# titus-leistner/mmlf

Hardware: AMD Instinct MI355X
Metric: 96x96 EPI patches/sec fwd+bwd, bs=512 (higher is better)
Workload: dtype f32 via 2 x f16 operand split (22 significant bits per operand, locally scaled; 3 MFMA passes, f32 accumulate)

## Files before the change

### include/mmlf_hip.h

```cpp
#ifndef MMLF_HIP_H
#define MMLF_HIP_H

#include <stddef.h>
#include <stdint.h>

#ifdef __cplusplus
extern "C" {
#endif

#define MMLF_TILE_POSITIONS 256

const char *mmlf_last_error(void);
#define MMLF_ABI_VERSION 10
int mmlf_abi_version(void);

const char *mmlf_build_info(void);
int mmlf_build_is_ablation(void);
int mmlf_conv_cus(void);

enum { MMLF_AUDIT_IN = 0, MMLF_AUDIT_PACKED = 1, MMLF_AUDIT_BIAS = 2, MMLF_AUDIT_OUT = 3, MMLF_AUDIT_REF = 4,
       MMLF_AUDIT_IN_AMAX = 5, MMLF_AUDIT_OUT_AMAX = 6, MMLF_AUDIT_BN_PARTIAL = 7, MMLF_AUDIT_MASK = 8, MMLF_AUDIT_CONV_N = 9 };
int mmlf_audit_conv_h2(int cs_in, int K, int N, int cs_out, int N_store, int out_shift, int cs_ref, int B, int H, int W,
                       int64_t *ends);
enum { MMLF_AUDIT_WG_IN = 0, MMLF_AUDIT_WG_G = 1, MMLF_AUDIT_WG_GW = 2, MMLF_AUDIT_WG_GB = 3, MMLF_AUDIT_WG_WORKSPACE = 4,
       MMLF_AUDIT_WG_IN_AMAX = 5, MMLF_AUDIT_WG_G_AMAX = 6, MMLF_AUDIT_WGRAD_N = 7 };
int mmlf_audit_wgrad_h2(int cs_in, int Cin, int cs_g, int Cout, int g_shift, int B, int H, int W, int64_t *ends);

int64_t mmlf_grid_alloc_positions(int B, int H, int W);
int64_t mmlf_packed_filter_floats(int K, int N);
int64_t mmlf_wgrad_workspace_floats(int Cin, int Cout, int B, int H, int W);

enum { MMLF_VAR_IDENTITY = 0, MMLF_VAR_TRANSPOSE = 1, MMLF_VAR_TRANSPOSE_FLIPH = 2 };

int mmlf_pack_filter(const float *w_oihw, float *packed, int Cout, int Cin, int variant, int dgrad,
                     void *stream);

int mmlf_conv2x2(const float *in, int cs_in, int K, const float *packed, const float *bias, int N,
                 float *out, int cs_out, int N_store, int out_shift, int vh, int vw,
                 int B, int H, int W, int relu, const float *relu_ref, int cs_ref, void *stream);

int64_t mmlf_packed_filter_split_bytes(int K, int N);
int mmlf_pack_filter_split(const float *w_oihw, void *packed, int Cout, int Cin, int variant, int dgrad,
                           void *stream);
int mmlf_conv2x2_split(const float *in, int cs_in, int K, const void *packed, const float *bias, int N,
                       float *out, int cs_out, int N_store, int out_shift, int vh, int vw,
                       int B, int H, int W, int relu, const float *relu_ref, int cs_ref, void *stream);
// ... 155 lines not shown
```

### mmlf_amd/_lib.py

```python
import ctypes
import os
import re

import torch

_HERE = os.path.dirname(os.path.abspath(__file__))
LIB_PATH = os.environ.get('MMLF_HIP_LIB') or os.path.join(_HERE, 'csrc', 'libmmlf_hip.so')

_HEADER = os.path.join(os.path.dirname(_HERE), 'include', 'mmlf_hip.h')
_CTYPES = {'int': ctypes.c_int, 'int32_t': ctypes.c_int32, 'int64_t': ctypes.c_int64, 'long long': ctypes.c_longlong,
           'double': ctypes.c_double, 'float': ctypes.c_float}


def signatures_from_header(text):
    text = re.sub(r'/\*.*?\*/', ' ', text, flags=re.S)
    text = re.sub(r'//[^\n]*', ' ', text)
    text = re.sub(r'^[ \t]*#(?:[^\n]*\\\n)*[^\n]*', ' ', text, flags=re.M)
    text = re.sub(r'\btypedef\s+struct\b[^{;]*\{[^{}]*\}[^;]*;', ' ', text)
    text = re.sub(r'\benum\b[^{;]*\{[^{}]*\}\s*;', ' ', text)
    text = re.sub(r'\bextern\s+"C"\s*\{', ' ', text).replace('}', ' ')

    def scalar(words, proto):
        key = ' '.join(w for w in words.split() if w != 'const')
        if key not in _CTYPES:
# ... 3 lines not shown
    sigs = {}
    for stmt in text.split(';'):
        proto = ' '.join(stmt.split())
        if not proto:
            continue
        m = re.fullmatch(r'([\w\s\*]+?)\b(\w+) ?\(([^()]*)\)', proto)
        if m is None or m.group(2) in sigs:
            raise ValueError(f'C header: cannot parse `{proto}`')
        ret, name, params = m.group(1), m.group(2), m.group(3).strip()
        if '*' in ret:
            if ret.split() != ['const', 'char', '*']:
                raise ValueError(f'C header: unknown return type `{ret.strip()}` in `{proto}`')
            res = ctypes.c_char_p
        else:
            res = scalar(ret, proto)
        args = []
        for param in ([] if params == 'void' else params.split(',')):
            d = re.fullmatch(r'\s*([\w\s\*]*?[\w\*])\s*\b(\w+)\s*((?:\[\w*\])?)\s*', param)
            if d is None or not re.search(r'\w', d.group(1)):
                raise ValueError(f'C header: cannot parse parameter `{param.strip()}` of `{proto}`')
            args.append(ctypes.c_void_p if '*' in d.group(1) or d.group(3) else scalar(d.group(1), proto))
        sigs[name] = (res, args)
    return sigs


def _header_text():
    with open(_HEADER) as f:
        return f.read()


SIGNATURES = signatures_from_header(_header_text())


def _header_abi_version():
    m = re.search(r'^#define\s+MMLF_ABI_VERSION\s+(\d+)', _header_text(), re.M)
    if m is None:
        raise RuntimeError(f'{_HEADER}: no MMLF_ABI_VERSION')
    return int(m.group(1))


ABI_VERSION = _header_abi_version()
_lib = None
BUILD_INFO = None


def validate(lib, path, environ=None):
    environ = os.environ if environ is None else environ
    got = lib.mmlf_abi_version() if hasattr(lib, 'mmlf_abi_version') else None
    if got != ABI_VERSION:
        raise RuntimeError(f'{path} implements ABI version {got}, this package needs {ABI_VERSION}: rebuild it '
                           'with `python -m mmlf_amd.csrc.build --force`')
    if not hasattr(lib, 'mmlf_build_info') or not hasattr(lib, 'mmlf_build_is_ablation'):
        raise RuntimeError(f'{path} does not say what it was built with (no mmlf_build_info): rebuild it')
    info = lib.mmlf_build_info()
    info = info.decode() if isinstance(info, bytes) else str(info)
    if lib.mmlf_build_is_ablation() and environ.get('MMLF_ALLOW_ABLATION') != '1':
        raise RuntimeError(f'{path} is a timing-ablation build that computes WRONG results ({info}); it is refused unless '
                           'MMLF_ALLOW_ABLATION=1 is set (unset MMLF_HIP_LIB to use the product library)')
    return info


def load():
    global _lib, BUILD_INFO
    if _lib is None:
        if not os.path.exists(LIB_PATH):
            raise RuntimeError(
                f'{LIB_PATH} not found: build it with `python -m mmlf_amd.csrc.build` '
                '(the HIP path has no CPU fallback)')
        lib = ctypes.CDLL(LIB_PATH)
        for name in ('mmlf_abi_version', 'mmlf_build_info', 'mmlf_build_is_ablation'):
            if hasattr(lib, name):
                getattr(lib, name).restype, getattr(lib, name).argtypes = SIGNATURES[name]
        BUILD_INFO = validate(lib, LIB_PATH)
        for name, (res, args) in SIGNATURES.items():
            fn = getattr(lib, name)
            fn.restype = res
            fn.argtypes = args
        _lib = lib
    return _lib


def build_info():
    load()
    return BUILD_INFO


def last_error():
    return load().mmlf_last_error().decode()


def call(name, *args):
    rc = getattr(load(), name)(*args)
    if rc != 0:
        raise RuntimeError(f'{name} failed: {last_error()}')


def ptr(t):
    return None if t is None else t.data_ptr()


def check(t, name, device, dtype=torch.float32, shape=None, numel=None, min_numel=None, contiguous=True):
    ok = (t is not None and t.device == device and dtype in (None, t.dtype) and (shape is None or tuple(t.shape) == tuple(shape))
          and (numel is None or t.numel() == numel) and (min_numel is None or t.numel() >= min_numel)
          and (not contiguous or t.is_contiguous()))
    if not ok:
        found = 'None' if t is None else f'{t.dtype} {tuple(t.shape)} on {t.device}, contiguous={t.is_contiguous()}'
        need = ', '.join(f'{k}={v}' for k, v in (('dtype', dtype), ('shape', shape if shape is None else tuple(shape)),
# ... 8 lines not shown
```

### mmlf_amd/csrc/build.py

```python
import os
import subprocess
import sys

HERE = os.path.dirname(os.path.abspath(__file__))
SOURCES = ['conv.hip', 'wgrad.hip', 'elementwise.hip']
LIB = os.path.join(HERE, 'libmmlf_hip.so')
HIPCC = os.environ.get('HIPCC', '/opt/rocm/bin/hipcc')
FLAGS = ['-O3', '--offload-arch=gfx950', '-fPIC', '-std=c++17', '-Wall', '-Wno-unused-function', '-ffp-contract=off']


def stale():
    if not os.path.exists(LIB):
        return True
    t = os.path.getmtime(LIB)
    deps = SOURCES + ['common.h', 'conv_device.h', 'build.py', os.path.join('..', '..', 'include', 'mmlf_hip.h')]
    return any(os.path.getmtime(os.path.join(HERE, d)) > t for d in deps)


def source_revision():
    root = os.path.dirname(os.path.dirname(HERE))
    try:
        rev = subprocess.check_output(['git', '-C', root, 'rev-parse', '--short=12', 'HEAD'], stderr=subprocess.DEVNULL).decode().strip()
        dirty = subprocess.call(['git', '-C', root, 'diff', '--quiet', 'HEAD', '--', 'mmlf_amd/csrc', 'include'],
                                stderr=subprocess.DEVNULL) != 0
        return rev + ('+' if dirty else '')
    except (OSError, subprocess.CalledProcessError):
        return 'unknown'


HASHED = SOURCES + ['common.h', 'conv_device.h', os.path.join('..', '..', 'include', 'mmlf_hip.h')]


def source_hash():
    import hashlib
    h = hashlib.sha1()
    for d in HASHED:
        with open(os.path.join(HERE, d), 'rb') as f:
            h.update(f.read())
    return h.hexdigest()[:12]


def build(force=False, verbose=True, extra_flags=(), lib=None):
    if lib is None and not extra_flags and not force and not stale():
        return LIB
    lib = lib or LIB
    tag = '' if lib == LIB else '.' + os.path.basename(lib).replace('.so', '')
    flags = [*FLAGS, f'-DMMLF_GIT_HASH="{source_revision()}"', f'-DMMLF_SRC_HASH="{source_hash()}"', *extra_flags]
    objs, jobs = [], []
    for src in SOURCES:
        obj = os.path.join(os.path.dirname(lib), src.replace('.hip', tag + '.o'))
        cmd = [HIPCC, *flags, '-c', os.path.join(HERE, src), '-o', obj]
        if verbose:
            print(' '.join(cmd), flush=True)
        jobs.append((cmd, subprocess.Popen(cmd)))
        objs.append(obj)
    failed = [cmd for cmd, job in jobs if job.wait() != 0]
    if failed:
        raise subprocess.CalledProcessError(1, failed[0])
    cmd = [HIPCC, '--offload-arch=gfx950', '-shared', '-fPIC', *objs, '-o', lib]
    if verbose:
        print(' '.join(cmd), flush=True)
    subprocess.check_call(cmd)
    return lib
# ... 10 lines not shown
```

### mmlf_amd/csrc/common.h

```cpp
#pragma once
#include <hip/hip_runtime.h>
#include <stdint.h>
#include <stdio.h>
#include <stdarg.h>
#include <mutex>

#define MMLF_TILE 256
#define MMLF_TILE_MAX 512

extern thread_local char g_mmlf_err[512];

static inline int mmlf_fail(const char *fmt, ...)
{
    va_list ap;
    va_start(ap, fmt);
    vsnprintf(g_mmlf_err, sizeof(g_mmlf_err), fmt, ap);
    va_end(ap);
    return 1;
}

#define MMLF_CHECK_ARG(cond, ...)                   \
    do {                                            \
        if (!(cond)) return mmlf_fail(__VA_ARGS__); \
    } while (0)

static inline int mmlf_launch_status(const char *what)
{
    hipError_t e = hipGetLastError();
    if (e != hipSuccess) return mmlf_fail("%s: launch failed: %s", what, hipGetErrorString(e));
    return 0;
}

static inline int current_device()
{
    int d = 0;
    if (hipGetDevice(&d) != hipSuccess || d < 0 || d >= 64) d = 0;
    return d;
}
struct PerDeviceOnce {
    std::once_flag flag[64];
    int status[64] = {};
    template <class F> int run(F &&f)
    {
        const int d = current_device();
        std::call_once(flag[d], [&] { status[d] = f(); });
        return status[d];
    }
};
static inline int mmlf_allow_lds(const void *kernel, size_t bytes, const char *what)
{
    const hipError_t e = hipFuncSetAttribute(kernel, hipFuncAttributeMaxDynamicSharedMemorySize, (int)bytes);
    if (e != hipSuccess)
        return mmlf_fail("%s: hipFuncSetAttribute(MaxDynamicSharedMemorySize = %zu) failed: %s", what, bytes, hipGetErrorString(e));
    return 0;
}

#ifdef MMLF_BOUNDS_DEBUG
static __device__ unsigned long long g_mmlf_oob[8];
#define MMLF_OOB(slot, cond) do { if (cond) atomicAdd(&g_mmlf_oob[slot], 1ull); } while (0)
#else
#define MMLF_OOB(slot, cond) do { } while (0)
#endif
enum { OOB_OUT = 0, OOB_IN = 1, OOB_WG_IN = 2, OOB_WG_G = 3, OOB_AMAX = 4, OOB_MASK = 5, OOB_WG_PART = 6, OOB_REF = 7 };

// ... 89 lines not shown
```

### mmlf_amd/csrc/elementwise.hip

```cpp
#include "common.h"
#include "../../include/mmlf_hip.h"

thread_local char g_mmlf_err[512] = "";

extern "C" const char *mmlf_last_error(void) { return g_mmlf_err; }
extern "C" int mmlf_abi_version(void) { return MMLF_ABI_VERSION; }
extern "C" int64_t mmlf_amax_entries(int B, int H, int W)
{
    if (B <= 0 || H <= 0 || W <= 0) return -1;
    return amax_entries(make_grid(B, H, W));
}
extern "C" int mmlf_grid_pad_w(void) { return GRID_PAD; }
extern "C" int mmlf_grid_pad_h(void) { return GRID_PAD; }
extern "C" int mmlf_amax_head(void) { return MMLF_AMAX_HEAD; }
extern "C" int mmlf_amax_shard_stride(void) { return MMLF_AMAX_SHARD_STRIDE; }
extern "C" int64_t mmlf_grid_alloc_positions(int B, int H, int W)
{
    if (B <= 0 || H <= 0 || W <= 0) return -1;
    return grid_alloc_positions(make_grid(B, H, W));
}
extern "C" int64_t mmlf_grid_alloc_positions_k3(int B, int H, int W)
{
    if (B <= 0 || H <= 0 || W <= 0) return -1;
    return grid_alloc_positions_k3(make_grid(B, H, W));
}

template <int V> struct VecIO;
template <> struct VecIO<4> {
    static __device__ __forceinline__ bool aligned(const float *p) { return (reinterpret_cast<uintptr_t>(p) & 15) == 0; }
    static __device__ __forceinline__ void load(const float *p, float *o)
    {
        if (aligned(p)) {
            const float4 v = *reinterpret_cast<const float4 *>(p);
            o[0] = v.x; o[1] = v.y; o[2] = v.z; o[3] = v.w;
// ... 1308 lines not shown
                                  int accumulate, float *coef, double *partial, int nblocks, int B, int H, int W,
                                  void *stream)
{
    MMLF_CHECK_ARG(gy && z && scale && shift && save_mean && save_invstd && coef && partial,
                   "mmlf_bn_bwd_reduce: null pointer");
    MMLF_CHECK_ARG(cs_gy % 2 == 0 && c_off % 2 == 0 && c_off >= 0 && cs_z % 4 == 0 && C > 0 && C <= cs_z &&
                       c_off + C <= cs_gy && (C + 3) / 4 <= 128,
                   "mmlf_bn_bwd_reduce: layout C=%d cs_z=%d cs_gy=%d c_off=%d", C, cs_z, cs_gy, c_off);
    MMLF_CHECK_ARG(nblocks > 0 && nblocks <= 4096, "mmlf_bn_bwd_reduce: nblocks=%d", nblocks);
    MMLF_CHECK_ARG(B > 0 && H > 0 && W > 0, "mmlf_bn_bwd_reduce: bad shape B=%d H=%d W=%d", B, H, W);
    hipStream_t st = (hipStream_t)stream;
    hipLaunchKernelGGL(bn_reduce_bwd_kernel, dim3(nblocks), dim3(256), 0, st, z, cs_z, gy, cs_gy, c_off,
                       scale, shift, save_mean, save_invstd, C, partial, B, H, W);
    hipLaunchKernelGGL(bn_bwd_finalize_kernel, dim3(C), dim3(64), 0, st, partial, nblocks, C,
                       (double)B * H * W, gamma, save_invstd, dgamma, dbeta, accumulate, coef);
    return mmlf_launch_status("mmlf_bn_bwd_reduce");
}

extern "C" int mmlf_bn_bwd_apply(const float *gy, int cs_gy, int c_off, const float *z, int cs_z, int C,
                                 const float *scale, const float *shift, const float *save_mean, const float *coef,
                                 float *dz, int cs_dz, int B, int H, int W, float *amax_out, void *stream)
{
    MMLF_CHECK_ARG(gy && z && scale && shift && save_mean && coef && dz, "mmlf_bn_bwd_apply: null pointer");
    MMLF_CHECK_ARG(cs_gy % 2 == 0 && c_off % 2 == 0 && c_off >= 0 && cs_z % 4 == 0 && cs_dz % 4 == 0 && C > 0 && C <= cs_z &&
                       C <= cs_dz && c_off + C <= cs_gy,
                   "mmlf_bn_bwd_apply: layout C=%d cs_z=%d cs_dz=%d cs_gy=%d c_off=%d", C, cs_z, cs_dz, cs_gy, c_off);
    MMLF_CHECK_ARG(B > 0 && H > 0 && W > 0, "mmlf_bn_bwd_apply: bad shape B=%d H=%d W=%d", B, H, W);
    const int nrows = B * (H + GRID_PAD);
    hipLaunchKernelGGL((bn_rows_kernel<1, 4>), dim3(nrows), dim3(256), 6 * (cs_dz + 4) * sizeof(float), (hipStream_t)stream, z, cs_z, gy,
                       cs_gy, c_off, scale, shift, save_mean, coef, C, dz, cs_dz, 0, cs_dz, H, W, amax_out, nrows);
    return mmlf_launch_status("mmlf_bn_bwd_apply");
}

static int relu_bwd_slice_args(const char *who, int cs_src, int c_off, int cs_ref, int ref_off, int C, int cs_dst, int B, int H,
                               int W)
{
    MMLF_CHECK_ARG(cs_src > 0 && cs_src % 2 == 0 && c_off % 2 == 0 && c_off >= 0 && cs_dst > 0 && cs_dst % 4 == 0 && C > 0 &&
                       C <= cs_dst && c_off + C <= cs_src && (C + 3) / 4 <= 128 && cs_dst / 4 <= 256,
                   "%s: layout C=%d cs_src=%d c_off=%d cs_dst=%d", who, C, cs_src, c_off, cs_dst);
    MMLF_CHECK_ARG(cs_ref > 0 && cs_ref % 2 == 0 && ref_off % 2 == 0 && ref_off >= 0 && ref_off + C <= cs_ref,
                   "%s: layout C=%d cs_ref=%d ref_off=%d", who, C, cs_ref, ref_off);
    MMLF_CHECK_ARG(B > 0 && H > 0 && W > 0, "%s: bad shape B=%d H=%d W=%d", who, B, H, W);
    return 0;
}

extern "C" int mmlf_relu_bwd_slice(const float *src, int cs_src, int c_off, const float *ref, int cs_ref, int ref_off, int C,
                                   float *dst, int cs_dst, int B, int H, int W, float *amax_out, void *stream)
{
    MMLF_CHECK_ARG(src && ref && dst, "mmlf_relu_bwd_slice: null pointer");
    if (relu_bwd_slice_args("mmlf_relu_bwd_slice", cs_src, c_off, cs_ref, ref_off, C, cs_dst, B, H, W)) return 1;
    const int nrows = B * (H + GRID_PAD);
    hipLaunchKernelGGL((relu_slice_rows_kernel<4>), dim3(nrows), dim3(256), 0, (hipStream_t)stream, src, cs_src, c_off, ref,
                       cs_ref, ref_off, C, dst, cs_dst, H, W, amax_out, nrows);
    return mmlf_launch_status("mmlf_relu_bwd_slice");
}

extern "C" int mmlf_audit_relu_bwd_slice(int cs_src, int c_off, int cs_ref, int ref_off, int C, int cs_dst, int B, int H, int W,
                                         int64_t *ends )
{
    MMLF_CHECK_ARG(ends, "mmlf_audit_relu_bwd_slice: null pointer");
    if (relu_bwd_slice_args("mmlf_audit_relu_bwd_slice", cs_src, c_off, cs_ref, ref_off, C, cs_dst, B, H, W)) return 1;
    const Grid g = make_grid(B, H, W);
    const long long q_last = ((long long)(B - 1) * g.R + H) * g.P + W;
    ends[MMLF_AUDIT_SLICE_SRC] = (q_last * cs_src + c_off + C) * 4;
    ends[MMLF_AUDIT_SLICE_REF] = (q_last * cs_ref + ref_off + C) * 4;
    ends[MMLF_AUDIT_SLICE_DST] = g.NQ * cs_dst * 4;
// ... 308 lines not shown
```

### mmlf_amd/csrc/wgrad.hip

```cpp
#include "conv_device.h"

#ifdef MMLF_BOUNDS_DEBUG
int mmlf_oob_counts_wgrad(unsigned long long *host8, int reset)
{
    if (hipMemcpyFromSymbol(host8, HIP_SYMBOL(g_mmlf_oob), sizeof(unsigned long long) * 8) != hipSuccess) return 1;
    if (reset) {
        const unsigned long long z[8] = {};
        if (hipMemcpyToSymbol(HIP_SYMBOL(g_mmlf_oob), z, sizeof(z)) != hipSuccess) return 1;
    }
    return 0;
}
#endif

struct WgradArgs {
    const float *in;
    const float *g;
    float *part;
    long long NQpad;
    int cs_in, cin, cs_g, g_shift, P, nsplit, nslice, chunks_per_split, nchunks;
    const float *in_amax, *g_amax;
    const float *chunk_scales;
    long long in_bytes, g_bytes, part_floats;
};

// ... 952 lines not shown
    }
}

static int thin_wgrad_waves() { return 4 * 4 * device_cus(); }

extern "C" int64_t mmlf_conv2x2_wgrad_thin_workspace_floats(int Cin)
{
    if (Cin <= 0) return -1;
    return (int64_t)thin_wgrad_waves() * 4 * (Cin + 1) * THIN_MAXN;
}

extern "C" int mmlf_conv2x2_wgrad_thin(const float *in, int cs_in, int Cin, const float *g, int cs_g, int Cout, int g_shift,
                                       float *gw_oihw, float *gb, int variant, int accumulate, float *workspace, int B,
                                       int H, int W, void *stream)
{
    MMLF_CHECK_ARG(in && g && gw_oihw && workspace, "mmlf_conv2x2_wgrad_thin: null pointer");
    MMLF_CHECK_ARG(Cout >= 1 && Cout <= THIN_MAXN && Cout <= cs_g && Cin >= 1 && Cin <= cs_in && cs_in % 4 == 0 && cs_in <= 512,
                   "mmlf_conv2x2_wgrad_thin: Cin=%d Cout=%d cs_in=%d", Cin, Cout, cs_in);
    MMLF_CHECK_ARG(B > 0 && H > 0 && W > 0 && variant >= 0 && variant <= 2, "mmlf_conv2x2_wgrad_thin: bad shape");
    const Grid gr = make_grid(B, H, W);
    MMLF_CHECK_ARG(g_shift >= 0 && g_shift <= gr.P + 1, "mmlf_conv2x2_wgrad_thin: g_shift=%d", g_shift);
    ThinArgs a = {};
    a.in = in; a.g = g; a.wpart = workspace; a.NQ = gr.NQ; a.npos = gr.NQ + gr.P + 2;
    a.cs_in = cs_in; a.C = Cin; a.N = Cout; a.cs_g = cs_g; a.g_shift = g_shift; a.P = gr.P; a.CIP = Cin + 1;
    hipStream_t st = (hipStream_t)stream;
    const int nwaves = thin_wgrad_waves();
    hipLaunchKernelGGL(thin_wgrad_kernel, dim3(nwaves / 4), dim3(256), 0, st, a);
    const int total = 4 * (Cin + 1) * Cout;
    hipLaunchKernelGGL(wgrad_reduce_wave_kernel, dim3((total + 3) / 4), dim3(256), 0, st, workspace, gw_oihw, gb, Cin, Cout,
                       Cin + 1, THIN_MAXN, nwaves, variant, accumulate);
    return mmlf_launch_status("mmlf_conv2x2_wgrad_thin");
}

extern "C" int mmlf_audit_wgrad_h2(int cs_in, int Cin, int cs_g, int Cout, int g_shift, int B, int H, int W,
                                   int64_t *ends )
{
    Wgrad16Cfg c;
    MMLF_CHECK_ARG(B > 0 && H > 0 && W > 0 && ends && Cin > 0 && Cout > 0, "mmlf_audit_wgrad_h2: bad argument");
    const Grid g = make_grid(B, H, W);
    const long long nchunks = g.NQpad / WG_KQ;
    MMLF_CHECK_ARG(wgrad16_cfg(Cin, Cout, nchunks, &c), "mmlf_audit_wgrad_h2: Cout=%d", Cout);
    const long long last_c = (nchunks - 1) * WG_KQ;
    ends[0] = (last_c + g.P + 32 + 1) * cs_in * 4;
    ends[1] = (last_c + g_shift + 31 + 1) * cs_g * 4;
    ends[2] = (int64_t)Cout * Cin * 4 * 4;
    ends[3] = (int64_t)Cout * 4;
    ends[4] = ((int64_t)c.nsplit * 4 * (c.nslice * 16 * c.mb) * (16 * c.nb)
               > wgrad_partial_floats(Cin, Cout) ? -1
               : wgrad_partial_floats(Cin, Cout) + 2 * nchunks + 2) * 4;
    ends[5] = (MMLF_AMAX_HEAD + amax_rows(g)) * 4;
    ends[6] = ends[5];
    return 0;
}

struct Wgrad9Cfg { int nt, nslice, nsplit; };
static inline bool wgrad9_cfg(int Cin, int Cout, Wgrad9Cfg *c)
{
    c->nt = pick_nt(Cout);
    if (c->nt < 0 || Cin <= 0) return false;
    c->nslice = 3 * ((Cin + 1 + 31) / 32);
    c->nsplit = wgrad_nsplit(c->nslice);
    return true;
}

extern "C" int64_t mmlf_wgrad3x3_workspace_floats(int Cin, int Cout, int B, int H, int W)
{
// ... 37 lines not shown
```

### mmlf_amd/engine.py

```python
import ctypes
import os
import threading

import torch

from . import _lib
from ._lib import call, check, ptr

VAR_IDENTITY, VAR_TRANSPOSE, VAR_TRANSPOSE_FLIPH = 0, 1, 2
BN_BLOCKS = 1024
LOSS_BLOCKS = 1024


def cs_of(c):
    return (c + 7) // 8 * 8


class Geometry:

    def __init__(self, B, H, W, ksize=2):
        self.B, self.H, self.W = B, H, W
        self.ksize = ksize
        self.P, self.R = W + int(_lib.load().mmlf_grid_pad_w()), H + int(_lib.load().mmlf_grid_pad_h())
        self.G = self.P * self.R
# ... 154 lines not shown

PROFILE = None


def _tic():
    e0, e1 = torch.cuda.Event(enable_timing=True), torch.cuda.Event(enable_timing=True)
    e0.record()
    return e0, e1


def _toc(events, tag, flops, nbytes):
    events[1].record()
    PROFILE.append((tag, flops, events[0], events[1], nbytes))


def _amax_of(geo, t, cs):
    a = getattr(t, 'absmax', None)
    if a is None:
        return geo.amax_of(t, cs)
    if CHECK_ABSMAX:
        true = geo.amax_of(t, cs)
        c = geo.amax_canonical(a)
        exact = geo.P >= 32
        bad = (c != true) if exact else (c < true)
        bad[0] = c[0] != true[0]
        if bool(bad.any()):
            k = int(bad.nonzero()[0])
            raise AssertionError(f'amax entry {k} holds {float(c[k])!r}, true max |x| is {float(true[k])!r}')
    return a


CHECK_ABSMAX = bool(os.environ.get('MMLF_CHECK_ABSMAX'))
OVERLAP_WGRAD = os.environ.get('MMLF_OVERLAP_WGRAD', '1') not in ('', '0')


CHECK_EXTENTS = bool(os.environ.get('MMLF_CHECK_EXTENTS'))
EXTENT_CHECKS = 0


def _audit(entry, scalars, n_ends, kind, have):
    global EXTENT_CHECKS
    ends = (ctypes.c_int64 * n_ends)()
    call(entry, *scalars, ends)
    for name, (k, t, off) in have.items():
        if t is None:
            continue
        got = t.untyped_storage().nbytes() - t.storage_offset() * t.element_size() - 4 * off
        if ends[k] > got:
            raise RuntimeError(f'MMLF_CHECK_EXTENTS: {kind}: the launch may touch {ends[k]} bytes behind `{name}`, '
                               f'the tensor has {got}')
    EXTENT_CHECKS += 1


def relu_bwd_slice(geo, src, cs_src, c_off, ref, cs_ref, ref_off, C, dst, cs_dst):
    amax = getattr(dst, 'absmax', None)
    if CHECK_EXTENTS:
        _audit('mmlf_audit_relu_bwd_slice', (cs_src, c_off, cs_ref, ref_off, C, cs_dst, geo.B, geo.H, geo.W), 4,
               f'relu_bwd_slice C={C} {cs_src}+{c_off} B={geo.B} {geo.H}x{geo.W}',
               {'src': (0, src, 0), 'ref': (1, ref, 0), 'dst': (2, dst, 0), 'amax': (3, amax, 0)})
    call('mmlf_relu_bwd_slice', ptr(src), cs_src, c_off, ptr(ref), cs_ref, ref_off, C, ptr(dst), cs_dst, geo.B, geo.H, geo.W,
         ptr(amax), _lib.stream_ptr())


THIN_MAX_N, THIN_MIN_K = 2, 64


# ... 328 lines not shown
            if packed is None:
                call('mmlf_pack_nchw', ptr(stacks[s]), cin0, ptr(x), cs_of(cin0), B, H, W, ptr(x.absmax), _lib.stream_ptr())
            cs_x = cs_of(cin0)
            recs = []
            x_relu, xmask = False, None
            for k, spec in enumerate(blocks):
                last = k == len(blocks) - 1
                x, cs_x, xmask = self._block_fwd(geo, spec, var, x, cs_x, x_relu, xmask, p, train, recs if save else None,
                                                 out=concat if last else None, cs_out=4 * self.chs, c_off=s * self.chs,
                                                 packs=packs, tracked=tracked, deferred=deferred if last else None, fold=fold)
                x_relu = relu_only
            tape['streams'].append(recs)
        if deferred:
            arr = lambda k: (ctypes.c_void_p * 4)(*[ptr(d[k]) for d in deferred])
            call('mmlf_bn_apply_relu4', arr(0), cs_of(self.chs), self.chs, arr(1), arr(2), ptr(concat), 4 * self.chs,
                 B, H, W, ptr(concat.absmax), _lib.stream_ptr())
            del deferred[:]
        if save and relu_only:
            tape['concat'] = concat
        x, cs_x, x_relu, xmask = concat, 4 * self.chs, False, None
        for spec in self.out_blocks:
            x, cs_x, xmask = self._block_fwd(geo, spec, VAR_IDENTITY, x, cs_x, x_relu, xmask, p, train,
                                             tape['out'] if save else None, packs=packs, tracked=tracked, fold=fold)
            x_relu = relu_only
        if tracked:
            counts = {}
            for t in tracked:
                counts.setdefault(t.data_ptr(), [t, 0])[1] += 1
            torch._foreach_add_([t for t, _ in counts.values()], [n for _, n in counts.values()])
        out = torch.empty((B, self.oc, H, W), dtype=torch.float32, device=dev)
        call('mmlf_unpack_nchw', ptr(x), cs_x, ptr(out), self.oc, B, H, W, _lib.stream_ptr())
        return out, (tape if save else None)

    def _block_bwd(self, geo, rec, p, grads, gy, cs_gy, c_off, need_dx, after_bn=None, overlap=False, packs=None):
        spec, var = rec.spec, rec.var
        dev = gy.device
        ws = _Workspace.get(dev)
        B, H, W = geo.B, geo.H, geo.W
        C, cs_mid = spec.cout, cs_of(spec.cout)
        x, cs_x, y, z = rec.x, rec.cs_x, rec.y, rec.z
        pre = spec.prefix
        sp = _lib.stream_ptr
        packs = packs or {}
        f16 = CONV_MODE == 'f16x3' and self.ksize == 2
        bn = rec.bn
        assert grads is None or rec.pk2d is None, 'a frozen forward (BatchNorm folded) has no parameter gradients'
        if grads is not None:
            gw1, gb1, gw2, gb2 = (grads[f'{pre}.{k}'] for k in ('0.weight', '0.bias', '2.weight', '2.bias'))

        y_relu = {'mask_in': rec.ymask} if rec.ymask is not None and f16 else {'ref': y, 'cs_ref': cs_mid}
        x_relu = {}
        if rec.x_relu:
            x_relu = {'mask_in': rec.xmask} if rec.xmask is not None and f16 else {'ref': x, 'cs_ref': cs_x}

        got = geo.bufs(([cs_mid] if bn else []) + [cs_mid] + ([cs_x] if need_dx else []), dev)
        dy = got[1 if bn else 0]
        dx = got[-1] if need_dx else None
        if bn:
            if grads is None and rec.eval:
                coef = torch.zeros(3 * C, dtype=torch.float32, device=dev)
                coef[:C].copy_(rec.scale)
            else:
                coef = torch.empty(3 * C, dtype=torch.float32, device=dev)
                if grads is None:
                    dgb = ws.scratch('bn_dgamma_dbeta', 2 * C)
                    dgamma, dbeta, acc = dgb[:C], dgb[C:2 * C], 0
                else:
                    dgamma, dbeta, acc = grads[f'{pre}.3.weight'], grads[f'{pre}.3.bias'], 1
                call('mmlf_bn_bwd_reduce', ptr(gy), cs_gy, c_off, ptr(z), cs_mid, C, ptr(rec.scale), ptr(rec.shift),
                     ptr(p[f'{pre}.3.weight']), ptr(rec.smean), ptr(rec.sinv), ptr(dgamma), ptr(dbeta), acc, ptr(coef),
                     ptr(ws.partial), BN_BLOCKS, B, H, W, sp())
                if rec.eval:
                    coef[C:].zero_()
            dz = got[0]
            call('mmlf_bn_bwd_apply', ptr(gy), cs_gy, c_off, ptr(z), cs_mid, C, ptr(rec.scale), ptr(rec.shift),
                 ptr(rec.smean), ptr(coef), ptr(dz), cs_mid, B, H, W, ptr(dz.absmax), sp())
        else:
            assert c_off == 0 and cs_gy == cs_mid
            dz = gy
        if after_bn:
            after_bn()
        if grads is not None:
            self._wgrad(geo, True, y, cs_mid, C, dz, cs_mid, C, gw2, gb2, var)
        pk2d = rec.pk2d if rec.pk2d is not None else self._packed(packs, p, f'{pre}.2.weight', var, True)
        self._dgrad(geo, True, dz, cs_mid, C, pk2d, C, dy, cs_mid, **y_relu)
        del dz, got
        if overlap and need_dx and grads is not None:
            self._dgrad(geo, False, dy, cs_mid, C, self._packed(packs, p, f'{pre}.0.weight', var, True), spec.cin, dx, cs_x,
                        **x_relu)
            main = torch.cuda.current_stream()
            ready = main.record_event()
            with torch.cuda.stream(ws.side):
                ws.side.wait_event(ready)
                self._wgrad(geo, False, x, cs_x, spec.cin, dy, cs_mid, C, gw1, gb1, var, side=True)
                done = ws.side.record_event()
            return dx, done, (x, dy)
        if grads is not None:
            self._wgrad(geo, False, x, cs_x, spec.cin, dy, cs_mid, C, gw1, gb1, var)
        if need_dx:
            self._dgrad(geo, False, dy, cs_mid, C, self._packed(packs, p, f'{pre}.0.weight', var, True), spec.cin, dx, cs_x,
                        **x_relu)
        return dx, None, None

    def backward(self, p, tape, grad_output, grads, on_done=None, input_grads=None):
        geo, dev = tape['geo'], tape['device']
        check(grad_output, 'grad_output', dev, shape=(geo.B, self.oc, geo.H, geo.W), contiguous=False)
        if grads is not None:
            self._check_dict('grads', grads, self._grad_names, dev)
        _Workspace.get(dev).enter_stream()
        B, H, W = geo.B, geo.H, geo.W
        cs = cs_of(self.oc)
        g = geo.buf(cs, dev)
        call('mmlf_pack_nchw', ptr(grad_output.contiguous()), self.oc, ptr(g), cs, B, H, W, ptr(g.absmax),
             _lib.stream_ptr())
        cs_g = cs
        want = [bool(w) for w in input_grads] if input_grads is not None else [False] * 4
        assert len(want) == 4
        dstacks = [None] * 4
        recs = tape['out']
        main = torch.cuda.current_stream()
        pending = None

        def settle():
            nonlocal pending
            if pending is not None:
                main.wait_event(pending[0])
                if on_done:
                    on_done(pending[1])
                pending = None

        while recs:
            rec = recs.pop()
            wide = OVERLAP_WGRAD and rec.spec.cin >= 128 and self.ksize == 2
            g, event, keep = self._block_bwd(geo, rec, p, grads, g, cs_g, 0, True, after_bn=settle, overlap=wide,
                                             packs=tape['packs'])
            settle()
            if event is not None:
                pending = (event, rec.spec.prefix, keep)
            elif on_done:
                on_done(rec.spec.prefix)
            cs_g = rec.cs_x
        for s in reversed(range(4)):
            recs = tape['streams'][s]
            if s == 2:
                settle()
            gs, cs_s, off = g, cs_g, s * self.chs
            if 'concat' in tape:
                cs_s, off = cs_of(self.chs), 0
                gs = geo.buf(cs_s, dev)
                relu_bwd_slice(geo, g, cs_g, s * self.chs, tape['concat'], cs_g, s * self.chs, self.chs, gs, cs_s)
            while recs:
                rec = recs.pop()
                gs, _, _ = self._block_bwd(geo, rec, p, grads, gs, cs_s, off, need_dx=bool(recs) or want[s],
                                           packs=tape['packs'])
                cs_s, off = rec.cs_x, 0
            if want[s]:
                dstacks[s] = torch.empty((B, self.views, 3, H, W), dtype=torch.float32, device=dev)
                call('mmlf_unpack_nchw', ptr(gs), cs_s, ptr(dstacks[s]), 3 * self.views, B, H, W, _lib.stream_ptr())
            if on_done and s in (2, 0):
                on_done('in_net_id' if s == 2 else 'in_net_hv')
        return dstacks
```

Before: 1149.

## Fuse head conv1 dgrad/wgrad into the preceding block's BN backward

When the final head block has no BN and a tiny output-channel count (1–2), its first 2x2 convolution's input gradient and weight gradient are no longer run as separate dgrad/wgrad passes. They are recomputed inside the next block's BN-backward reduce and apply kernels, which read the thin head gradient directly and rebuild the relu-masked gradient per channel. This removes a full-size intermediate gradient write and read, plus several kernel launches. The cost is extra per-element FMAs in both kernels, an extra wgrad-partials reduction, and new ABI entry points enabled by default through an environment flag.

```diff
diff --git a/include/mmlf_hip.h b/include/mmlf_hip.h
--- a/include/mmlf_hip.h
+++ b/include/mmlf_hip.h
@@ -11,7 +11,7 @@
 #define MMLF_TILE_POSITIONS 256
 
 const char *mmlf_last_error(void);
-#define MMLF_ABI_VERSION 10
+#define MMLF_ABI_VERSION 11
 int mmlf_abi_version(void);
 
 const char *mmlf_build_info(void);
diff --git a/include/mmlf_hip_ext.h b/include/mmlf_hip_ext.h
--- /dev/null
+++ b/include/mmlf_hip_ext.h
@@ -0,0 +1,27 @@
+#ifndef MMLF_HIP_EXT_H
+#define MMLF_HIP_EXT_H
+
+#include "mmlf_hip.h"
+
+#ifdef __cplusplus
+extern "C" {
+#endif
+
+int mmlfx_head_bn_bwd_reduce(const float *z, int cs_z, int C, const float *scale, const float *shift,
+                            const float *gamma, const float *save_mean, const float *save_invstd,
+                            const float *dyh, int cs_g, int oc, int g_shift, const float *w_oihw, int variant,
+                            float *dgamma, float *dbeta, float *coef, double *partial, int nblocks,
+                            float *gw_oihw, float *gb, int accumulate, float *workspace,
+                            int B, int H, int W, void *stream);
+int mmlfx_head_bn_bwd_apply(const float *z, int cs_z, int C, const float *scale, const float *shift,
+                           const float *save_mean, const float *coef, const float *dyh, int cs_g, int oc, int g_shift,
+                           const float *w_oihw, int variant, float *dz, int cs_dz, int B, int H, int W,
+                           float *amax_out , void *stream);
+enum { MMLF_AUDIT_HEAD_Z = 0, MMLF_AUDIT_HEAD_DYH = 1, MMLF_AUDIT_HEAD_W = 2, MMLF_AUDIT_HEAD_DZ = 3, MMLF_AUDIT_HEAD_AMAX = 4,
+       MMLF_AUDIT_HEAD_PARTIAL = 5, MMLF_AUDIT_HEAD_WORKSPACE = 6, MMLF_AUDIT_HEAD_N = 7 };
+int mmlfx_audit_head_bn_bwd(int cs_z, int C, int cs_g, int oc, int cs_dz, int nblocks, int B, int H, int W, int64_t *ends);
+
+#ifdef __cplusplus
+}
+#endif
+#endif
diff --git a/mmlf_amd/_lib.py b/mmlf_amd/_lib.py
--- a/mmlf_amd/_lib.py
+++ b/mmlf_amd/_lib.py
@@ -59,6 +59,11 @@
 SIGNATURES = signatures_from_header(_header_text())
 
 
+_HEADER_EXT = os.path.join(os.path.dirname(_HERE), 'include', 'mmlf_hip_ext.h')
+with open(_HEADER_EXT) as _f:
+    EXT_SIGNATURES = signatures_from_header(_f.read())
+
+
 def _header_abi_version():
     m = re.search(r'^#define\s+MMLF_ABI_VERSION\s+(\d+)', _header_text(), re.M)
     if m is None:
@@ -99,7 +104,7 @@
             if hasattr(lib, name):
                 getattr(lib, name).restype, getattr(lib, name).argtypes = SIGNATURES[name]
         BUILD_INFO = validate(lib, LIB_PATH)
-        for name, (res, args) in SIGNATURES.items():
+        for name, (res, args) in list(SIGNATURES.items()) + list(EXT_SIGNATURES.items()):
             fn = getattr(lib, name)
             fn.restype = res
             fn.argtypes = args
diff --git a/mmlf_amd/csrc/build.py b/mmlf_amd/csrc/build.py
--- a/mmlf_amd/csrc/build.py
+++ b/mmlf_amd/csrc/build.py
@@ -13,7 +13,8 @@
     if not os.path.exists(LIB):
         return True
     t = os.path.getmtime(LIB)
-    deps = SOURCES + ['common.h', 'conv_device.h', 'build.py', os.path.join('..', '..', 'include', 'mmlf_hip.h')]
+    deps = SOURCES + ['common.h', 'conv_device.h', 'build.py', os.path.join('..', '..', 'include', 'mmlf_hip.h'),
+            os.path.join('..', '..', 'include', 'mmlf_hip_ext.h')]
     return any(os.path.getmtime(os.path.join(HERE, d)) > t for d in deps)
 
 
@@ -28,7 +29,8 @@
         return 'unknown'
 
 
-HASHED = SOURCES + ['common.h', 'conv_device.h', os.path.join('..', '..', 'include', 'mmlf_hip.h')]
+HASHED = SOURCES + ['common.h', 'conv_device.h', os.path.join('..', '..', 'include', 'mmlf_hip.h'),
+                    os.path.join('..', '..', 'include', 'mmlf_hip_ext.h')]
 
 
 def source_hash():
diff --git a/mmlf_amd/csrc/common.h b/mmlf_amd/csrc/common.h
--- a/mmlf_amd/csrc/common.h
+++ b/mmlf_amd/csrc/common.h
@@ -30,6 +30,10 @@
     if (e != hipSuccess) return mmlf_fail("%s: launch failed: %s", what, hipGetErrorString(e));
     return 0;
 }
+
+int mmlf_thin_wgrad_partials_fit(const char *who, int nsplit, int np);
+int mmlf_thin_wgrad_reduce_partials(const float *workspace, float *gw_oihw, float *gb, int Cin, int Cout, int np, int nsplit,
+                                    int variant, int accumulate, hipStream_t st);
 
 static inline int current_device()
 {
diff --git a/mmlf_amd/csrc/elementwise.hip b/mmlf_amd/csrc/elementwise.hip
--- a/mmlf_amd/csrc/elementwise.hip
+++ b/mmlf_amd/csrc/elementwise.hip
@@ -1,5 +1,6 @@
 #include "common.h"
 #include "../../include/mmlf_hip.h"
+#include "../../include/mmlf_hip_ext.h"
 
 thread_local char g_mmlf_err[512] = "";
 
@@ -1374,6 +1375,306 @@
     return mmlf_launch_status("mmlf_bn_bwd_apply");
 }
 
+template <int OC>
+__device__ __forceinline__ void head_load_dyh(const float *__restrict__ dyh, int cs_g, size_t p, int P, float (&d)[4][OC])
+{
+    const size_t q[4] = {p, p - 1, p - P, p - P - 1};
+#pragma unroll
+    for (int t = 0; t < 4; ++t) {
+        const float *gp = dyh + q[t] * cs_g;
+        if (OC == 2) {
+            const float2 v = *reinterpret_cast<const float2 *>(gp);
+            d[t][0] = v.x; d[t][OC - 1] = v.y;
+        } else {
+            d[t][0] = *gp;
+        }
+    }
+}
+
+template <int OC>
+__device__ __forceinline__ float head_gy(const float (&w)[4][OC], const float (&d)[4][OC])
+{
+    float gy = 0.f;
+#pragma unroll
+    for (int t = 0; t < 4; ++t)
+#pragma unroll
+        for (int o = 0; o < OC; ++o) gy = fmaf(w[t][o], d[t][o], gy);
+    return gy;
+}
+
+template <int OC>
+__global__ __launch_bounds__(256)
+void head_fused_reduce_kernel(const float *__restrict__ z, int cs_z, int C, const float *__restrict__ scale,
+                              const float *__restrict__ shift, const float *__restrict__ mean, const float *__restrict__ invstd,
+                              const float *__restrict__ dyh, int cs_g, const float *__restrict__ w1, int variant,
+                              double *__restrict__ partial, float *__restrict__ wpart, int B, int H, int W)
+{
+    const int P = W + GRID_PAD, R = H + GRID_PAD;
+    const int cvn = (C + 3) / 4, Cpad = 4 * cvn;
+    const int ppi = 256 / cvn;
+    const int tid = threadIdx.x;
+    const int pl = tid / cvn, cg = tid - pl * cvn;
+    const bool active = pl < ppi;
+    __shared__ double red[2][256][4];
+    extern __shared__ float head_stage[];
+    for (int c = tid; c < Cpad; c += 256) {
+        const bool in = c < C;
+        head_stage[0 * Cpad + c] = in ? scale[c] : 0.f;
+        head_stage[1 * Cpad + c] = in ? shift[c] : 0.f;
+        head_stage[2 * Cpad + c] = in ? mean[c] : 0.f;
+        head_stage[3 * Cpad + c] = in ? invstd[c] : 0.f;
+#pragma unroll
+        for (int t = 0; t < 4; ++t)
+#pragma unroll
+            for (int o = 0; o < OC; ++o)
+                head_stage[(4 + t * OC + o) * Cpad + c] = in ? w1[((size_t)o * C + c) * 4 + master_tap<2>(t, variant)] : 0.f;
+    }
+    __syncthreads();
+    float sc[4], sh[4], mu[4], iv[4], w[4][4][OC];
+#pragma unroll
+    for (int e = 0; e < 4; ++e) {
+        const int c = 4 * cg + e;
+        sc[e] = head_stage[0 * Cpad + c]; sh[e] = head_stage[1 * Cpad + c];
+        mu[e] = head_stage[2 * Cpad + c]; iv[e] = head_stage[3 * Cpad + c];
+#pragma unroll
+        for (int t = 0; t < 4; ++t)
+#pragma unroll
+            for (int o = 0; o < OC; ++o) w[e][t][o] = head_stage[(4 + t * OC + o) * Cpad + c];
+    }
+    double s0[4], s1[4];
+    float acc[4][4][OC];
+    float gsum[OC];
+#pragma unroll
+    for (int e = 0; e < 4; ++e) {
+        s0[e] = 0; s1[e] = 0;
+#pragma unroll
+        for (int t = 0; t < 4; ++t)
+#pragma unroll
+            for (int o = 0; o < OC; ++o) acc[e][t][o] = 0.f;
+    }
+#pragma unroll
+    for (int o = 0; o < OC; ++o) gsum[o] = 0.f;
+    const int nrows = B * H;
+    const bool z_aligned = (reinterpret_cast<uintptr_t>(z) & 15) == 0;
+    for (int row = blockIdx.x; row < nrows; row += gridDim.x) {
+        const int b = row / H, y = row - b * H + 1;
+        const size_t base = ((size_t)(b * R + y) * P + 1);
+        for (int x = pl; active && x < W; x += ppi) {
+            const size_t p = base + x;
+            float zz[4], d[4][OC];
+            VecIO<4>::load_nt(z + p * cs_z + 4 * cg, zz, z_aligned);
+            head_load_dyh<OC>(dyh, cs_g, p, P, d);
+            if (cg == 0) {
+#pragma unroll
+                for (int o = 0; o < OC; ++o) {
+                    float s = d[3][o];
+                    if (x == W - 1) s += d[2][o];
+                    if (y == H) s += d[1][o];
+                    if (x == W - 1 && y == H) s += d[0][o];
+                    gsum[o] += s;
+                }
+            }
+#pragma unroll
+            for (int e = 0; e < 4; ++e) {
+                const float u = fmaf(zz[e], sc[e], sh[e]);
+                const float out = fmaxf(u, 0.f);
+                const float g = u > 0.f ? head_gy<OC>(w[e], d) : 0.f;
+                s0[e] += g;
+                s1[e] += (double)g * (double)((zz[e] - mu[e]) * iv[e]);
+#pragma unroll
+                for (int t = 0; t < 4; ++t)
+#pragma unroll
+                    for (int o = 0; o < OC; ++o) acc[e][t][o] = fmaf(out, d[t][o], acc[e][t][o]);
+            }
+        }
+    }
+#pragma unroll
+    for (int e = 0; e < 4; ++e) { red[0][tid][e] = s0[e]; red[1][tid][e] = s1[e]; }
+    __syncthreads();
+    if (tid < cvn) {
+#pragma unroll
+        for (int e = 0; e < 4; ++e) {
+            double a0 = 0, a1 = 0;
+            for (int p = 0; p < ppi; ++p) { a0 += red[0][p * cvn + tid][e]; a1 += red[1][p * cvn + tid][e]; }
+            const int c = 4 * tid + e;
+            if (c < C) {
+                partial[((size_t)blockIdx.x * 2 + 0) * C + c] = a0;
+                partial[((size_t)blockIdx.x * 2 + 1) * C + c] = a1;
+            }
+        }
+    }
+    __syncthreads();
+    float *fr = reinterpret_cast<float *>(&red[0][0][0]);
+    float *pp = wpart + (size_t)blockIdx.x * 4 * (C + 1) * OC;
+#pragma unroll
+    for (int t = 0; t < 4; ++t) {
+#pragma unroll
+        for (int e = 0; e < 4; ++e)
+#pragma unroll
+            for (int o = 0; o < OC; ++o) fr[tid * (4 * OC) + e * OC + o] = acc[e][t][o];
+        __syncthreads();
+        if (tid < cvn) {
+#pragma unroll
+            for (int e = 0; e < 4; ++e)
+#pragma unroll
+                for (int o = 0; o < OC; ++o) {
+                    float a = 0.f;
+                    for (int p = 0; p < ppi; ++p) a += fr[(p * cvn + tid) * (4 * OC) + e * OC + o];
+                    const int c = 4 * tid + e;
+                    if (c < C) pp[((size_t)t * (C + 1) + c) * OC + o] = a;
+                }
+        }
+        __syncthreads();
+    }
+    if (cg == 0)
+#pragma unroll
+        for (int o = 0; o < OC; ++o) fr[pl * OC + o] = gsum[o];
+    __syncthreads();
+    if (tid < OC) {
+        float a = 0.f;
+        for (int p = 0; p < ppi; ++p) a += fr[p * OC + tid];
+#pragma unroll
+        for (int t = 0; t < 4; ++t) pp[((size_t)t * (C + 1) + C) * OC + tid] = t == 0 ? a : 0.f;
+    }
+}
+
+template <int OC>
+__global__ __launch_bounds__(256)
+void head_fused_rows_kernel(const float *__restrict__ z, int cs_z, const float *__restrict__ dyh, int cs_g,
+                            const float *__restrict__ w1, int variant, const float *__restrict__ scale,
+                            const float *__restrict__ shift, const float *__restrict__ mean, const float *__restrict__ coef,
+                            int C, float *__restrict__ out, int cs_out, int H, int W, float *__restrict__ amax, int nrows)
+{
+    extern __shared__ float coefs[];
+    const int P = W + GRID_PAD, R = H + GRID_PAD;
+    const int cvn = cs_out / 4;
+    const int Cpad = cs_out;
+    for (int c = threadIdx.x; c < Cpad; c += blockDim.x) {
+        const bool ok = c < C;
+        coefs[c] = ok ? scale[c] : 0.f;
+        coefs[Cpad + c] = ok ? shift[c] : 0.f;
+        coefs[2 * Cpad + c] = ok ? mean[c] : 0.f;
+        coefs[3 * Cpad + c] = ok ? coef[c] : 0.f;
+        coefs[4 * Cpad + c] = ok ? coef[C + c] : 0.f;
+        coefs[5 * Cpad + c] = ok ? coef[2 * C + c] : 0.f;
+#pragma unroll
+        for (int t = 0; t < 4; ++t)
+#pragma unroll
+            for (int o = 0; o < OC; ++o)
+                coefs[(6 + t * OC + o) * Cpad + c] = ok ? w1[((size_t)o * C + c) * 4 + master_tap<2>(t, variant)] : 0.f;
+    }
+    __syncthreads();
+    const int dx = 256 / cvn, dc = 256 - dx * cvn;
+    for (int row = blockIdx.x; row < nrows; row += gridDim.x) {
+        const int y = row % R;
+        const size_t base = (size_t)row * P;
+        const bool row_in = (y >= 1 && y <= H);
+        int x = threadIdx.x / cvn, cg = threadIdx.x - x * cvn;
+        float mx = 0.f;
+        for (; x < P; x += dx, cg += dc) {
+            if (cg >= cvn) { cg -= cvn; ++x; if (x >= P) break; }
+            float o[4] = {0.f, 0.f, 0.f, 0.f};
+            if (row_in && x >= 1 && x <= W && 4 * cg < C) {
+                float zz[4], d[4][OC];
+                VecIO<4>::load_nt(z + (base + x) * cs_z + 4 * cg, zz);
+                head_load_dyh<OC>(dyh, cs_g, base + x, P, d);
+#pragma unroll
+                for (int k = 0; k < 4; ++k) {
+                    const int c = 4 * cg + k;
+                    float w[4][OC];
+#pragma unroll
+                    for (int t = 0; t < 4; ++t)
+#pragma unroll
+                        for (int oo = 0; oo < OC; ++oo) w[t][oo] = coefs[(6 + t * OC + oo) * Cpad + c];
+                    const float u = fmaf(zz[k], coefs[c], coefs[Cpad + c]);
+                    const float g = u > 0.f ? head_gy<OC>(w, d) : 0.f;
+                    o[k] = coefs[3 * Cpad + c] * g - coefs[4 * Cpad + c] - coefs[5 * Cpad + c] * (zz[k] - coefs[2 * Cpad + c]);
+                }
+            }
+#pragma unroll
+            for (int k = 0; k < 4; ++k) mx = fmaxf(mx, fabsf(o[k]));
+            VecIO<4>::store_nt(out + (base + x) * cs_out + 4 * cg, o);
+        }
+        if (amax) mmlf_amax_update_row(mx, amax, row);
+    }
+}
+
+static int head_bn_bwd_args(const char *who, int cs_z, int C, int cs_g, int oc, int g_shift, int variant, int B, int H, int W)
+{
+    MMLF_CHECK_ARG(cs_z > 0 && cs_z % 4 == 0 && C > 0 && C <= cs_z && (C + 3) / 4 <= 128, "%s: layout C=%d cs_z=%d", who, C, cs_z);
+    MMLF_CHECK_ARG(oc >= 1 && oc <= 2 && oc <= cs_g && (oc == 1 || cs_g % 2 == 0), "%s: oc=%d cs_g=%d (oc <= 2)", who, oc, cs_g);
+    MMLF_CHECK_ARG(g_shift == 0, "%s: g_shift=%d (the gradient of a pad-1 convolution: 0)", who, g_shift);
+    MMLF_CHECK_ARG(variant >= 0 && variant <= 2, "%s: variant=%d", who, variant);
+    MMLF_CHECK_ARG(B > 0 && H > 0 && W > 0, "%s: bad shape B=%d H=%d W=%d", who, B, H, W);
+    MMLF_CHECK_ARG(make_grid(B, H, W).NQ < (1ll << 31), "%s: batch x image too large", who);
+    return 0;
+}
+
+extern "C" int mmlfx_head_bn_bwd_reduce(const float *z, int cs_z, int C, const float *scale, const float *shift,
+                                       const float *gamma, const float *save_mean, const float *save_invstd, const float *dyh,
+                                       int cs_g, int oc, int g_shift, const float *w_oihw, int variant, float *dgamma,
+                                       float *dbeta, float *coef, double *partial, int nblocks, float *gw_oihw, float *gb,
+                                       int accumulate, float *workspace, int B, int H, int W, void *stream)
+{
+    MMLF_CHECK_ARG(z && scale && shift && save_mean && save_invstd && dyh && w_oihw && coef && partial && gw_oihw && workspace,
+                   "mmlfx_head_bn_bwd_reduce: null pointer");
+    if (head_bn_bwd_args("mmlfx_head_bn_bwd_reduce", cs_z, C, cs_g, oc, g_shift, variant, B, H, W)) return 1;
+    MMLF_CHECK_ARG((reinterpret_cast<uintptr_t>(dyh) & 7) == 0, "mmlfx_head_bn_bwd_reduce: dyh is not 8-byte aligned");
+    MMLF_CHECK_ARG(nblocks > 0 && nblocks <= 4096, "mmlfx_head_bn_bwd_reduce: nblocks=%d", nblocks);
+    if (mmlf_thin_wgrad_partials_fit("mmlfx_head_bn_bwd_reduce", nblocks, oc)) return 1;
+    hipStream_t st = (hipStream_t)stream;
+    const size_t lds = (size_t)(4 + 4 * oc) * ((C + 3) / 4 * 4) * sizeof(float);
+    if (oc == 1)
+        hipLaunchKernelGGL(head_fused_reduce_kernel<1>, dim3(nblocks), dim3(256), lds, st, z, cs_z, C, scale, shift, save_mean,
+                           save_invstd, dyh, cs_g, w_oihw, variant, partial, workspace, B, H, W);
+    else
+        hipLaunchKernelGGL(head_fused_reduce_kernel<2>, dim3(nblocks), dim3(256), lds, st, z, cs_z, C, scale, shift, save_mean,
+                           save_invstd, dyh, cs_g, w_oihw, variant, partial, workspace, B, H, W);
+    hipLaunchKernelGGL(bn_bwd_finalize_kernel, dim3(C), dim3(64), 0, st, partial, nblocks, C,
+                       (double)B * H * W, gamma, save_invstd, dgamma, dbeta, accumulate, coef);
+    if (mmlf_thin_wgrad_reduce_partials(workspace, gw_oihw, gb, C, oc, oc, nblocks, variant, accumulate, st)) return 1;
+    return mmlf_launch_status("mmlfx_head_bn_bwd_reduce");
+}
+
+extern "C" int mmlfx_head_bn_bwd_apply(const float *z, int cs_z, int C, const float *scale, const float *shift,
+                                      const float *save_mean, const float *coef, const float *dyh, int cs_g, int oc,
+                                      int g_shift, const float *w_oihw, int variant, float *dz, int cs_dz, int B, int H, int W,
+                                      float *amax_out, void *stream)
+{
+    MMLF_CHECK_ARG(z && scale && shift && save_mean && coef && dyh && w_oihw && dz, "mmlfx_head_bn_bwd_apply: null pointer");
+    if (head_bn_bwd_args("mmlfx_head_bn_bwd_apply", cs_z, C, cs_g, oc, g_shift, variant, B, H, W)) return 1;
+    MMLF_CHECK_ARG(cs_dz % 4 == 0 && C <= cs_dz && cs_dz <= 512, "mmlfx_head_bn_bwd_apply: C=%d cs_dz=%d", C, cs_dz);
+    MMLF_CHECK_ARG((reinterpret_cast<uintptr_t>(dyh) & 7) == 0, "mmlfx_head_bn_bwd_apply: dyh is not 8-byte aligned");
+    const int nrows = B * (H + GRID_PAD);
+    const size_t lds = (size_t)(6 + 4 * oc) * cs_dz * sizeof(float);
+    hipStream_t st = (hipStream_t)stream;
+    if (oc == 1)
+        hipLaunchKernelGGL(head_fused_rows_kernel<1>, dim3(nrows), dim3(256), lds, st, z, cs_z, dyh, cs_g, w_oihw, variant, scale,
+                           shift, save_mean, coef, C, dz, cs_dz, H, W, amax_out, nrows);
+    else
+        hipLaunchKernelGGL(head_fused_rows_kernel<2>, dim3(nrows), dim3(256), lds, st, z, cs_z, dyh, cs_g, w_oihw, variant, scale,
+                           shift, save_mean, coef, C, dz, cs_dz, H, W, amax_out, nrows);
+    return mmlf_launch_status("mmlfx_head_bn_bwd_apply");
+}
+
+extern "C" int mmlfx_audit_head_bn_bwd(int cs_z, int C, int cs_g, int oc, int cs_dz, int nblocks, int B, int H, int W,
+                                      int64_t *ends )
+{
+    MMLF_CHECK_ARG(ends, "mmlfx_audit_head_bn_bwd: null pointer");
+    if (head_bn_bwd_args("mmlfx_audit_head_bn_bwd", cs_z, C, cs_g, oc, 0, 0, B, H, W)) return 1;
+    MMLF_CHECK_ARG(cs_dz % 4 == 0 && C <= cs_dz && nblocks > 0, "mmlfx_audit_head_bn_bwd: C=%d cs_dz=%d nblocks=%d", C, cs_dz, nblocks);
+    const Grid g = make_grid(B, H, W);
+    const long long q_last = ((long long)(B - 1) * g.R + H) * g.P + W;
+    ends[MMLF_AUDIT_HEAD_Z] = (q_last * cs_z + (C + 3) / 4 * 4) * 4;
+    ends[MMLF_AUDIT_HEAD_DYH] = (q_last * cs_g + oc) * 4;
+    ends[MMLF_AUDIT_HEAD_W] = (int64_t)oc * C * 4 * 4;
+    ends[MMLF_AUDIT_HEAD_DZ] = g.NQ * cs_dz * 4;
+    ends[MMLF_AUDIT_HEAD_AMAX] = (MMLF_AMAX_HEAD + (long long)B * g.R) * 4;
+    ends[MMLF_AUDIT_HEAD_PARTIAL] = (int64_t)nblocks * 2 * C * 8;
+    ends[MMLF_AUDIT_HEAD_WORKSPACE] = (int64_t)nblocks * 4 * (C + 1) * oc * 4;
+    return 0;
+}
+
 static int relu_bwd_slice_args(const char *who, int cs_src, int c_off, int cs_ref, int ref_off, int C, int cs_dst, int B, int H,
                                int W)
 {
diff --git a/mmlf_amd/csrc/wgrad.hip b/mmlf_amd/csrc/wgrad.hip
--- a/mmlf_amd/csrc/wgrad.hip
+++ b/mmlf_amd/csrc/wgrad.hip
@@ -1008,6 +1008,23 @@
     return mmlf_launch_status("mmlf_conv2x2_wgrad_thin");
 }
 
+int mmlf_thin_wgrad_partials_fit(const char *who, int nsplit, int np)
+{
+    MMLF_CHECK_ARG(nsplit > 0 && np >= 1 && np <= THIN_MAXN && (long long)nsplit * np <= (long long)thin_wgrad_waves() * THIN_MAXN,
+                   "%s: %d partials of %d columns do not fit the thin weight gradient's workspace (%d of %d)", who, nsplit, np,
+                   thin_wgrad_waves(), THIN_MAXN);
+    return 0;
+}
+
+int mmlf_thin_wgrad_reduce_partials(const float *workspace, float *gw_oihw, float *gb, int Cin, int Cout, int np, int nsplit,
+                                    int variant, int accumulate, hipStream_t st)
+{
+    const int total = 4 * (Cin + 1) * Cout;
+    hipLaunchKernelGGL(wgrad_reduce_wave_kernel, dim3((total + 3) / 4), dim3(256), 0, st, workspace, gw_oihw, gb, Cin, Cout,
+                       Cin + 1, np, nsplit, variant, accumulate);
+    return 0;
+}
+
 extern "C" int mmlf_audit_wgrad_h2(int cs_in, int Cin, int cs_g, int Cout, int g_shift, int B, int H, int W,
                                    int64_t *ends )
 {
diff --git a/mmlf_amd/engine.py b/mmlf_amd/engine.py
--- a/mmlf_amd/engine.py
+++ b/mmlf_amd/engine.py
@@ -210,6 +210,7 @@
 
 CHECK_ABSMAX = bool(os.environ.get('MMLF_CHECK_ABSMAX'))
 OVERLAP_WGRAD = os.environ.get('MMLF_OVERLAP_WGRAD', '1') not in ('', '0')
+HEAD_FUSED = os.environ.get('MMLF_HEAD_FUSED', '1') not in ('', '0')
 
 
 CHECK_EXTENTS = bool(os.environ.get('MMLF_CHECK_EXTENTS'))
@@ -604,9 +605,10 @@
         call('mmlf_unpack_nchw', ptr(x), cs_x, ptr(out), self.oc, B, H, W, _lib.stream_ptr())
         return out, (tape if save else None)
 
-    def _block_bwd(self, geo, rec, p, grads, gy, cs_gy, c_off, need_dx, after_bn=None, overlap=False, packs=None):
+    def _block_bwd(self, geo, rec, p, grads, gy, cs_gy, c_off, need_dx, after_bn=None, overlap=False, packs=None,
+                   leave_conv1=False, head=None):
         spec, var = rec.spec, rec.var
-        dev = gy.device
+        dev = rec.x.device
         ws = _Workspace.get(dev)
         B, H, W = geo.B, geo.H, geo.W
         C, cs_mid = spec.cout, cs_of(spec.cout)
@@ -628,7 +630,25 @@
         got = geo.bufs(([cs_mid] if bn else []) + [cs_mid] + ([cs_x] if need_dx else []), dev)
         dy = got[1 if bn else 0]
         dx = got[-1] if need_dx else None
-        if bn:
+        if bn and head is not None:
+            assert grads is not None and not rec.eval and gy is None and self.ksize == 2
+            coef = torch.empty(3 * C, dtype=torch.float32, device=dev)
+            dz = got[0]
+            hws = ws.scratch('thin_wgrad', int(_lib.load().mmlf_conv2x2_wgrad_thin_workspace_floats(C)))
+            if CHECK_EXTENTS:
+                _audit('mmlfx_audit_head_bn_bwd', (cs_mid, C, head['cs'], head['oc'], cs_mid, BN_BLOCKS, B, H, W), 7,
+                       f'head_bn_bwd C={C} oc={head["oc"]} B={B} {H}x{W}',
+                       {'z': (0, z, 0), 'dyh': (1, head['dy'], 0), 'w_oihw': (2, head['w'], 0), 'dz': (3, dz, 0),
+                        'amax': (4, dz.absmax, 0), 'partial': (5, ws.partial, 0), 'workspace': (6, hws, 0)})
+            call('mmlfx_head_bn_bwd_reduce', ptr(z), cs_mid, C, ptr(rec.scale), ptr(rec.shift), ptr(p[f'{pre}.3.weight']),
+                 ptr(rec.smean), ptr(rec.sinv), ptr(head['dy']), head['cs'], head['oc'], 0, ptr(head['w']), head['var'],
+                 ptr(grads[f'{pre}.3.weight']), ptr(grads[f'{pre}.3.bias']), ptr(coef), ptr(ws.partial), BN_BLOCKS,
+                 ptr(head['gw']), ptr(head['gb']), 1, ptr(hws), B, H, W, sp())
+            head['done']()
+            call('mmlfx_head_bn_bwd_apply', ptr(z), cs_mid, C, ptr(rec.scale), ptr(rec.shift), ptr(rec.smean), ptr(coef),
+                 ptr(head['dy']), head['cs'], head['oc'], 0, ptr(head['w']), head['var'], ptr(dz), cs_mid, B, H, W,
+                 ptr(dz.absmax), sp())
+        elif bn:
             if grads is None and rec.eval:
                 coef = torch.zeros(3 * C, dtype=torch.float32, device=dev)
                 coef[:C].copy_(rec.scale)
@@ -657,6 +677,8 @@
         pk2d = rec.pk2d if rec.pk2d is not None else self._packed(packs, p, f'{pre}.2.weight', var, True)
         self._dgrad(geo, True, dz, cs_mid, C, pk2d, C, dy, cs_mid, **y_relu)
         del dz, got
+        if leave_conv1:
+            return dy, None, None
         if overlap and need_dx and grads is not None:
             self._dgrad(geo, False, dy, cs_mid, C, self._packed(packs, p, f'{pre}.0.weight', var, True), spec.cin, dx, cs_x,
                         **x_relu)
@@ -701,11 +723,24 @@
                     on_done(pending[1])
                 pending = None
 
+        head = None
         while recs:
             rec = recs.pop()
             wide = OVERLAP_WGRAD and rec.spec.cin >= 128 and self.ksize == 2
+            spec = rec.spec
+            fuse = (HEAD_FUSED and spec.bn is None and grads is not None and self.ksize == 2 and spec.cout <= THIN_MAX_N
+                    and spec.cin >= THIN_MIN_K and rec.cs_x <= 512 and bool(recs) and recs[-1].bn is True
+                    and not recs[-1].eval and recs[-1].z is not None)
+            if fuse:
+                dy, _, _ = self._block_bwd(geo, rec, p, grads, g, cs_g, 0, False, packs=tape['packs'], leave_conv1=True)
+                head = {'dy': dy, 'cs': cs_of(spec.cout), 'oc': spec.cout, 'w': p[f'{spec.prefix}.0.weight'], 'var': rec.var,
+                        'gw': grads[f'{spec.prefix}.0.weight'], 'gb': grads[f'{spec.prefix}.0.bias'],
+                        'done': (lambda prefix=spec.prefix: on_done(prefix)) if on_done else (lambda: None)}
+                g, cs_g = None, rec.cs_x
+                continue
             g, event, keep = self._block_bwd(geo, rec, p, grads, g, cs_g, 0, True, after_bn=settle, overlap=wide,
-                                             packs=tape['packs'])
+                                             packs=tape['packs'], head=head)
+            head = None
             settle()
             if event is not None:
                 pending = (event, rec.spec.prefix, keep)
```

Result: no change. 1157, median of 6 (+0.7%).
